# angelvillar96/STLPose

Hardware: AMD Instinct MI355X
Metric: images/sec/GPU HRNet-W32 384x288 train step; PCKh@0.5 parity (higher is better)
Workload: dtype f16/bf16; 1 GPU; HRNet-W32 384x288 bs=32/GPU train step (fwd+MSE+bwd+Adam), random-init weights; global_batch=32, parallelism=dp1

## Files before the change

stlpose_amd/csrc/conv_core.hip:

```cpp
#include <stdlib.h>
#include <algorithm>
#include <cstring>
#include <type_traits>
#include "common.cuh"

#ifndef STL_DT
#define STL_DT 2
#endif
#define STL_HAS_F32 (STL_DT == 0 || STL_DT == 2)
#define STL_HAS_BF16 (STL_DT == 1 || STL_DT == 2)
#define STL_HAS_F16 (STL_DT == 3 || STL_DT == 2)

struct ConvK {
    stl_conv p;
    int tiles_c, npt;
    int HR, HC, HP;
    int PI, pad, seff;
    int nchunks, wres;
    int cipad;
    int off_cs, off_cm, off_a, off_b, off_red;
    int sz_a, sz_b;
    int TH, TW;
    int dbg;
    float r_HC, r_TW, r_tc, r_PI, r_vp;
// ... 554 lines not shown
    STL_LAUNCH((conv_core_kernel<T, KS, WM, WN, MT, NTW, NVA, Q, PE, OCC, WR, ZM, TY, DB, EO>), grid, dim3(64 * WM * WN), lds, st, k);
    static char nbuf[160];
    static const char* nm = stl_kname<T>(nbuf, "conv_core_kernel", {KS, WM, WN, MT, NTW, NVA, Q, PE, OCC, WR, ZM, stl_code<TY>(), DB, EO});
    stl_note_kernel(nm, true);
    STL_LAUNCH_CHECK("conv_core");
    return 0;
}

struct Shape {
    int px, co, thr;
    int ws;
    int lthr, nva_max;
};
constexpr int NSHAPES = 11;
constexpr Shape SHAPES[NSHAPES] = {{128, 64, 256, 0, 256, 9}, {512, 32, 512, 0, 512, 6}, {256, 64, 512, 0, 512, 3},
                                   {256, 64, 512, 2, 512, 3}, {128, 32, 256, 0, 256, 6},
                                   {256, 64, 512, 3, 512, 3}, {128, 64, 512, 3, 512, 2}, {128, 64, 512, 1, 256, 9},
                                   {256, 32, 512, 0, 512, 3}, {128, 32, 512, 1, 256, 3}, {256, 32, 512, 3, 512, 3}};

template <typename T, typename TY, int KS, bool Q, bool PE, int EO = -1>
int dispatch(int shape, int nva, const ConvK& k, dim3 grid, size_t lds, hipStream_t st) {
    constexpr int EOC = (KS == 3 && (Q || EO == 48)) ? EO : -1;
    constexpr int EOW = (KS == 3 && EO != 48) ? EO : -1;
    switch (shape) {
        case 0:
            if (nva <= 3) return launch<T, TY, KS, 4, 1, 2, 4, 3, Q, PE>(k, grid, lds, st);
            if (nva <= 9) return launch<T, TY, KS, 4, 1, 2, 4, 9, Q, PE>(k, grid, lds, st);
            break;
        case 1:
            if (nva <= 6) return launch<T, TY, KS, 8, 1, 4, 2, 6, Q, PE>(k, grid, lds, st);
            break;
        case 2:
            if (nva <= 3) return launch<T, TY, KS, 4, 2, 4, 2, 3, Q, PE, 1>(k, grid, lds, st);
            break;
        case 3:
            if constexpr (KS == 3) {
                if (nva <= 3 && !k.wres) return launch<T, TY, KS, 4, 2, 4, 2, 3, Q, PE, 1, 0, false, true, EOC>(k, grid, lds, st);
            }
            break;
        case 8:
            if (nva <= 3 && k.wres) return launch<T, TY, KS, 8, 1, 2, 2, 3, Q, PE, 4, 1, false, false, EOC>(k, grid, lds, st);
            if (nva <= 3) return launch<T, TY, KS, 8, 1, 2, 2, 3, Q, PE, (Q ? 3 : 4)>(k, grid, lds, st);
            break;
        case 4:
            if (nva <= 3 && k.wres) return launch<T, TY, KS, 4, 1, 2, 2, 3, Q, PE, 4, 1>(k, grid, lds, st);
            if (nva <= 3) return launch<T, TY, KS, 4, 1, 2, 2, 3, Q, PE, (Q ? 3 : 4)>(k, grid, lds, st);
            if (nva <= 6) return launch<T, TY, KS, 4, 1, 2, 2, 6, Q, PE, 3>(k, grid, lds, st);
            break;
        case 7:
            if (nva <= 3) return launch_ws<T, TY, KS, 2, 4, 3, Q, (Q ? -1 : EOW)>(k, grid, lds, st);
            if (nva <= 9) return launch_ws<T, TY, KS, 2, 4, 9, Q, (Q ? -1 : EOW)>(k, grid, lds, st);
            break;
        case 9:
            if (nva <= 3) return launch_ws<T, TY, KS, 2, 2, 3, Q, EOW>(k, grid, lds, st);
            break;
    }
    return stl_set_error("conv: no kernel variant for block shape %d with %d staging vectors per thread", shape, nva);
}

static bool bnadd_shape_ok(int shape, int nva) { return nva <= 3 && (shape == 0 || shape == 2 || shape == 3 || shape == 4 || shape == 5 || shape == 6 || shape == 8 || shape == 10); }
template <typename T>
int dispatch_bnadd(int shape, int nva, const ConvK& k, dim3 grid, size_t lds, hipStream_t st) {
    if (nva <= 3) switch (shape) {
        case 0: return launch<T, T, 3, 4, 1, 2, 4, 3, true, true, 1, -1, true>(k, grid, lds, st);
        case 2:
        case 3: return launch<T, T, 3, 4, 2, 4, 2, 3, true, true, 1, -1, true>(k, grid, lds, st);
        case 4: return launch<T, T, 3, 4, 1, 2, 2, 3, true, true, 3, -1, true>(k, grid, lds, st);
        case 8: return launch<T, T, 3, 8, 1, 2, 2, 3, true, true, 3, -1, true>(k, grid, lds, st);
    }
    return stl_set_error("conv: no block-end (BNADD) variant for block shape %d with %d staging vectors per thread", shape, nva);
}

template <typename T, typename TY>
int conv_backend(int path, const stl_conv& p, const ConvK& k, int shape, int nva, dim3 grid, size_t lds, hipStream_t st) {
    const bool q = p.src.mode == STL_SRC_BNBWD;
    if constexpr (!std::is_same<T, TY>::value) {
        if (!q) return stl_set_error("conv: ydtype differs from dtype, but the launch is not a data gradient (BNBWD source)");
    }
    if constexpr (std::is_same<T, f16>::value) {
        if (q) return stl_set_error("conv: STL_F16 is a forward-tensor type; gradients are bf16 (dtype STL_BF16 + ydtype STL_F16)");
    }
    constexpr bool FWD = std::is_same<T, TY>::value, BWD = !std::is_same<T, f16>::value;
    if (path == 0) return run_1x1<T, TY>(p, st);
    if (path == 3) {
        if constexpr (sizeof(T) == 2) return dispatch_r2<T, TY>(p, k, shape == 5 ? 0 : (shape == 6 ? 1 : 2), grid, lds, st);
        return stl_set_error("conv_r2: 16-bit element types only");
    }
    if (path == 1) {
        if constexpr (FWD) return dispatch_bnadd<T>(shape, nva, k, grid, lds, st);
    }
    const bool plain = !p.bias && !p.addend && !p.mask_y && !p.mask_z && !p.red;
    const char* noeo = getenv("STL_CONV_NO_EO");
    const int eo = (noeo && (atoi(noeo) & 1)) ? -1 : epi_code(p);
    if (p.ks == 3) {
        if (q) {
            if constexpr (BWD) {
                if (eo == 1) return dispatch<T, TY, 3, true, false, 1>(shape, nva, k, grid, lds, st);
                if (eo == 7) return dispatch<T, TY, 3, true, false, 7>(shape, nva, k, grid, lds, st);
                if (eo == 2) return dispatch<T, TY, 3, true, false, 2>(shape, nva, k, grid, lds, st);
                if (eo == 0) return dispatch<T, TY, 3, true, false, 0>(shape, nva, k, grid, lds, st);
                return dispatch<T, TY, 3, true, false>(shape, nva, k, grid, lds, st);
            }
        }
        if constexpr (FWD) {
            if (plain && eo == 8) return dispatch<T, T, 3, false, true, 8>(shape, nva, k, grid, lds, st);
            if (!plain && eo == 48) return dispatch<T, T, 3, false, false, 48>(shape, nva, k, grid, lds, st);
            return plain ? dispatch<T, T, 3, false, true>(shape, nva, k, grid, lds, st) : dispatch<T, T, 3, false, false>(shape, nva, k, grid, lds, st);
        }
    }
    if (q) {
        if constexpr (BWD) return dispatch<T, TY, 1, true, false>(shape, nva, k, grid, lds, st);
    }
    if constexpr (FWD) return plain ? dispatch<T, T, 1, false, true>(shape, nva, k, grid, lds, st) : dispatch<T, T, 1, false, false>(shape, nva, k, grid, lds, st);
    return stl_set_error("conv: no kernel for this dtype combination");
}

struct Plan {
    int shape, TH, TW;
    size_t lds;
    double cost;
};

size_t lds_bytes(const stl_conv& p, int shape, int TH, int TW, int ck, ConvK* out) {
    const int taps = p.ks * p.ks, seff = p.stride;
    const int HR = (TH - 1) * seff + p.ks, HC = (TW - 1) * seff + p.ks;
    const int nchunks = ceil_div(p.Ci, ck), cipad = nchunks * ck;
    const int bco = SHAPES[shape].co, ws = SHAPES[shape].ws;
    if (ws == 3) {
        int off = 3 * cipad * 4;
        const int off_cm = off;
        off = (off + 4 * bco * 4 + 15) & ~15;
        const int off_a = off, pl = ((HR * HC * R2_PS) + 15) & ~15;
        off += 2 * pl;
        const int off_b = (off + 1023) & ~1023;
        off = off_b + bco * R2_ROWF;
        const int off_red = off;
        off += 512 * 4;
        if (out) {
            out->HR = HR, out->HC = HC, out->HP = HR * HC, out->nchunks = nchunks, out->cipad = cipad;
            out->off_cs = 0, out->off_cm = off_cm, out->off_a = off_a, out->off_b = off_b, out->off_red = off_red;
            out->sz_a = pl, out->sz_b = 0, out->wres = 0;
        }
        return (size_t)off;
    }
    int off = 3 * cipad * 4;
    const int off_cm = off;
    off += 4 * bco * 4;
    off = (off + 15) & ~15;
    const int off_a = off;
    const int sz_a = ((HR * HC * PSA) + 15) & ~15;
    off += sz_a * (ws ? 2 : 1);
    const int off_b = off;
    const int sz_b = bco * (taps * 64 + 32);
    const bool resident = nchunks == 1 || (ws == 1 && (size_t)off + (size_t)sz_b * nchunks <= 150 * 1024);
    off += resident ? sz_b * nchunks : sz_b * (ws ? 2 : 1);
    const int off_red = off_a;
    const int red = 8 * 2 * bco * 4;
    if (off - off_a < red) off = off_a + red;
    if (out) {
        out->HR = HR, out->HC = HC, out->HP = HR * HC, out->nchunks = nchunks, out->cipad = cipad;
        out->off_cs = 0, out->off_cm = off_cm, out->off_a = off_a, out->off_b = off_b, out->off_red = off_red;
        out->sz_a = ws ? sz_a : 0, out->sz_b = (ws && !resident) ? sz_b : 0;
        out->wres = resident ? 1 : 0;
    }
    return (size_t)off;
}

Plan choose_plan(const stl_conv& p, int ck) {
    Plan best{-1, 0, 0, 0, 1e300};
    const int vrows = p.B * (p.Ho + 1);
    const int r2_env = getenv("STL_CONV_R2") ? atoi(getenv("STL_CONV_R2")) : 11;
    const bool deep_small = p.stride == 1 && p.ks == 3 && p.Co >= 256 && (int64_t)p.B * p.Ho * p.Wo <= 16384 &&
                            !((r2_env & 8) && p.dtype != STL_F32 && p.Ci % 32 == 0 && p.Ci >= 64 && (r2_env & (p.src.mode == STL_SRC_BNBWD ? 2 : 1)));
    const bool want_ws = p.stride == 2 || deep_small;
    const bool wide_k = p.Co <= 32 && p.Ci >= 128 && p.stride == 1 && p.ks == 3 && !p.stuff && (int64_t)p.B * p.Ho * p.Wo >= 65536;
    const bool c32 = p.Co <= 32 && p.stride == 1 && p.ks == 3 && !wide_k;
    for (int shape = 0; shape < NSHAPES; ++shape) {
        const Shape sh = SHAPES[shape];
        if (sh.px == 0) continue;
        if (sh.px > 128 && p.stride == 2) continue;
        if ((sh.ws == 1) != want_ws) continue;
        if (want_ws && shape != (deep_small ? 9 : 7)) continue;
        if (shape == 2 || shape == 3 || shape == 5 || shape == 6) {
            static const bool db_on = !(getenv("STL_CONV_DB") && atoi(getenv("STL_CONV_DB")) == 0);
            const int r2_mode = r2_env;
            const bool db = db_on && p.ks == 3 && p.stride == 1 && p.Ci > ck;
            const bool dgrad = p.src.mode == STL_SRC_BNBWD;
            const bool r2 = db && (r2_mode & (dgrad ? 2 : 1)) && p.dtype != STL_F32 && p.Ci % 32 == 0 && p.Ci >= 64;
            const bool small_map = (r2_mode & 8) && p.Co >= 256 && (int64_t)p.B * p.Ho * p.Wo <= 16384;
            const int want = r2 ? ((dgrad || (r2_mode & 4) || small_map) ? 6 : 5) : (db ? 3 : 2);
            if (shape != want) continue;
        }
        if ((shape == 1 || shape == 8 || shape == 10) && p.Co > 32) continue;
        if ((shape == 4 || shape == 8 || shape == 10) && !c32) continue;
        if (c32 && shape != 4 && shape != 8 && shape != 10) continue;
        {
            const bool r2c32 = (r2_env & 16) && p.dtype != STL_F32 && p.Ci == 32 && (r2_env & (p.src.mode == STL_SRC_BNBWD ? 2 : 1));
            if (c32 && (shape == 8 || shape == 10) && (shape == 10) != r2c32) continue;
        }
        if (wide_k && shape != 1) continue;
        const int nblk_co = ceil_div(p.Co, sh.co);
        for (int tw = (p.Wo < 4 ? p.Wo : 4); tw <= p.Wo && tw <= sh.px; ++tw)
          for (int frac = 4; frac >= 1; --frac) {
            int th = (sh.px / tw) * frac / 4;
            if (th > vrows) th = vrows;
            if (th < 1) continue;
            const int hr = (th - 1) * p.stride + p.ks, hc = (tw - 1) * p.stride + p.ks;
            const int nva = ceil_div(hr * hc * 4, sh.lthr);
            if (nva > sh.nva_max) continue;
            const size_t lds = lds_bytes(p, shape, th, tw, ck, nullptr);
            if (shape == 4 && lds > 40 * 1024 && nva <= 3) continue;
            if (shape == 8 && lds > 80 * 1024) continue;
            if ((shape == 5 || shape == 6 || shape == 10) && lds > 76 * 1024) continue;
            if (lds > 158 * 1024) continue;
            const double tiles = (double)ceil_div(vrows, th) * ceil_div(p.Wo, tw);
            const double mfma = tiles * sh.px * sh.co * nblk_co * (double)p.Ci * p.ks * p.ks / 2048.0;
            const double bytes = tiles * nblk_co * ((double)hr * hc * p.Ci + (double)sh.co * p.ks * p.ks * p.Ci) * 2.0 / 12.0;
            const double blocks = tiles * nblk_co;
            double cost = (mfma > bytes ? mfma : bytes) + 0.3 * (mfma < bytes ? mfma : bytes);
            const double waves = blocks * sh.thr / 64.0;
            if (waves < 2048.0) cost *= 1.0 + 0.15 * (2048.0 / waves - 1.0 > 4.0 ? 4.0 : 2048.0 / waves - 1.0);
            if (c32 && shape == 4) cost *= 4.0;
            if (shape == 5 || shape == 6 || shape == 10) cost *= 0.98;
            if (cost < best.cost) best = Plan{shape, th, tw, lds, cost};
        }
    }
    return best;
}

}

#if STL_HAS_BF16
static int ydtype_of(const stl_conv& p) { return (p.dtype == STL_BF16 && p.ydtype == STL_F16) ? STL_F16 : p.dtype; }
int stl_conv_backend_bf16(int path, const stl_conv& p, const ConvK& k, int shape, int nva, dim3 grid, size_t lds, hipStream_t st) {
    if (ydtype_of(p) == STL_F16) return conv_backend<__bf16, f16>(path, p, k, shape, nva, grid, lds, st);
    return conv_backend<__bf16, __bf16>(path, p, k, shape, nva, grid, lds, st);
}
#endif
#if STL_HAS_F32
int stl_conv_backend_f32(int path, const stl_conv& p, const ConvK& k, int shape, int nva, dim3 grid, size_t lds, hipStream_t st) {
    return conv_backend<float, float>(path, p, k, shape, nva, grid, lds, st);
}
#endif
#if STL_HAS_F16
int stl_conv_backend_f16(int path, const stl_conv& p, const ConvK& k, int shape, int nva, dim3 grid, size_t lds, hipStream_t st) {
    return conv_backend<f16, f16>(path, p, k, shape, nva, grid, lds, st);
}
#endif
// ... 2 lines not shown
#ifdef STL_STAMPS
extern "C" int stl_debug_conv_stamps(long long* host12) {
    return hipMemcpyFromSymbol(host12, HIP_SYMBOL(g_stamps), 14 * sizeof(long long)) == hipSuccess ? 0 : stl_set_error("stamps: copy failed");
}
extern "C" int stl_debug_conv_stamps2(long long* host64) {
    return hipMemcpyFromSymbol(host64, HIP_SYMBOL(g_stamps2), 64 * sizeof(long long)) == hipSuccess ? 0 : stl_set_error("stamps: copy failed");
}
#endif

extern "C" int stl_conv_plan(stl_conv* pp) {
    stl_conv& p = *pp;
    STL_CHECK(p.dtype == STL_F32 || p.dtype == STL_BF16 || p.dtype == STL_F16, "conv_plan: bad dtype");
    STL_CHECK((p.ks == 1 || p.ks == 3) && (p.stride == 1 || p.stride == 2) && p.Ci > 0 && p.Co > 0, "conv_plan: bad geometry");
    const int ck = p.dtype == STL_F32 ? 16 : 32;
    Plan plan = choose_plan(p, ck);
    STL_CHECK(plan.shape >= 0, "conv_plan: no tile fits LDS for %dx%d ks %d stride %d Ci %d", p.Ho, p.Wo, p.ks, p.stride, p.Ci);
    p.shape = plan.shape, p.TH = plan.TH, p.TW = plan.TW;
    return 0;
}

extern "C" int stl_conv_bnadd_ok(const stl_conv* pp) {
    const stl_conv& p = *pp;
    if (use_1x1(p)) return 1;
    if (!(p.ks == 3 && p.stride == 1 && !p.stuff && p.shape >= 0 && p.shape < NSHAPES && p.TH > 0 && p.TW > 0)) return 0;
    const Shape sh = SHAPES[p.shape];
    const int nva = ceil_div((p.TH + 2) * (p.TW + 2) * 4, sh.lthr);
    return bnadd_shape_ok(p.shape, nva) ? 1 : 0;
}

extern "C" int stl_conv_forward(const stl_conv* pp, void* stream) {
    const stl_conv& p = *pp;
    STL_CHECK(p.dtype == STL_F32 || p.dtype == STL_BF16 || p.dtype == STL_F16, "conv: bad dtype %d", p.dtype);
    STL_CHECK(p.ydtype == 0 || p.ydtype == p.dtype || (p.dtype == STL_BF16 && p.ydtype == STL_F16), "conv: ydtype %d does not go with dtype %d", p.ydtype, p.dtype);
    STL_CHECK(p.ks == 1 || p.ks == 3, "conv: ks must be 1 or 3 (got %d)", p.ks);
    STL_CHECK(p.stride == 1 || p.stride == 2, "conv: stride must be 1 or 2");
    STL_CHECK(!(p.stuff && p.stride != 1), "conv: stuff requires stride 1");
    STL_CHECK(!(p.ks == 1 && (p.stride != 1 || p.stuff)), "conv: 1x1 must be stride 1");
    const int kv = p.dtype == STL_F32 ? 4 : 8, ck = 4 * kv;
    STL_CHECK(p.Ci % kv == 0 && p.Ci > 0, "conv: Ci=%d must be a multiple of %d", p.Ci, kv);
    STL_CHECK(p.Co % 8 == 0 && p.Co > 0, "conv: Co=%d must be a multiple of 8", p.Co);
    STL_CHECK(p.B > 0 && p.Hi > 0 && p.Wi > 0 && p.Ho > 0 && p.Wo > 0, "conv: empty tensor");
    STL_CHECK((int64_t)p.B * p.Hi * p.Wi * p.Ci < (1ll << 31) && (int64_t)p.B * p.Ho * p.Wo * p.Co < (1ll << 31),
              "conv: tensors of 2^31 or more elements are not supported");
    const int pad = p.ks == 3 ? 1 : 0;
    if (p.stuff) {
        STL_CHECK((p.Ho + 1) / 2 == p.Hi && (p.Wo + 1) / 2 == p.Wi, "conv(stuff): %dx%d is not the stride-2 image of %dx%d", p.Hi, p.Wi, p.Ho, p.Wo);
    } else {
        STL_CHECK((p.Hi + 2 * pad - p.ks) / p.stride + 1 == p.Ho && (p.Wi + 2 * pad - p.ks) / p.stride + 1 == p.Wo,
                  "conv: output %dx%d inconsistent with input %dx%d ks %d stride %d", p.Ho, p.Wo, p.Hi, p.Wi, p.ks, p.stride);
    }
    STL_CHECK(p.src.x && p.w && p.out, "conv: null tensor pointer");
    STL_CHECK(p.src.mode >= 0 && p.src.mode <= 3, "conv: bad src mode");
    const bool zm = p.src.mode == STL_SRC_BNADD;
    STL_CHECK(!zm || (((p.ks == 3 && p.stride == 1 && !p.stuff) || use_1x1(p)) && p.src.y && p.src.beta && (p.src.stats || (p.src.rmean && p.src.rvar))),
              "conv: a BNADD source needs a 3x3 stride-1 (or wide 1x1) convolution, the skip tensor in src.y and BatchNorm parameters");
    STL_CHECK(zm || !p.src_out, "conv: src_out needs a BNADD source");
    STL_CHECK(!zm || (!p.bias && !p.addend && !p.mask_y && !p.mask_z && !p.red), "conv: a BNADD source takes no epilogue operands");
    STL_CHECK(p.src.mode == STL_SRC_PLAIN || p.src.gamma, "conv: BN source without gamma");
    STL_CHECK(p.src.mode != STL_SRC_BN || p.src.beta, "conv: BN source without beta");
    STL_CHECK(p.src.mode != STL_SRC_BN || p.src.stats || (p.src.rmean && p.src.rvar), "conv: BN source without statistics");
    STL_CHECK(p.src.mode != STL_SRC_BNBWD || (p.src.y && (p.src.stats || (p.src.rmean && p.src.rvar)) && p.src.rstats), "conv: BNBWD source incomplete");
    STL_CHECK(!(p.out_stats && p.red), "conv: out_stats and red are exclusive");
    STL_CHECK(!p.red || p.mask_y, "conv: red needs mask_y");
    STL_CHECK(!p.mask_y || (p.mask_bn.gamma && p.mask_bn.beta && (p.mask_bn.stats || (p.mask_bn.rmean && p.mask_bn.rvar))), "conv: mask BN incomplete");

    const auto backend = p.dtype == STL_BF16 ? stl_conv_backend_bf16 : (p.dtype == STL_F16 ? stl_conv_backend_f16 : stl_conv_backend_f32);
    if (use_1x1(p))
        return backend(0, p, ConvK{}, 0, 0, dim3(1), 0, (hipStream_t)stream);

    Plan plan;
    if (p.shape >= 0 && p.shape < NSHAPES && p.TH > 0 && p.TW > 0) {
        STL_CHECK(p.TH * p.TW <= SHAPES[p.shape].px, "conv: tile %dx%d exceeds block shape %d", p.TH, p.TW, p.shape);
        plan = Plan{p.shape, p.TH, p.TW, 0, 0.0};
    } else if (p.TH > 0 && p.TW > 0) {
        STL_CHECK(p.TH * p.TW <= 128, "conv: explicit tile %dx%d exceeds 128 pixels", p.TH, p.TW);
        plan = Plan{0, p.TH, p.TW, 0, 0.0};
    } else {
        plan = choose_plan(p, ck);
        STL_CHECK(plan.shape >= 0, "conv: no tile fits LDS for %dx%d ks %d stride %d Ci %d", p.Ho, p.Wo, p.ks, p.stride, p.Ci);
    }
    if (plan.shape == 5 && !r2_takes(p, 0)) plan.shape = 3;
    if (plan.shape == 6 && !r2_takes(p, 1)) plan.shape = 0;
    if (plan.shape == 10 && !r2_takes(p, 2)) plan.shape = 8;
    {
        const Shape shp = SHAPES[plan.shape];
        const int nv = ceil_div(((plan.TH - 1) * p.stride + p.ks) * ((plan.TW - 1) * p.stride + p.ks) * 4, shp.lthr);
        STL_CHECK(nv <= shp.nva_max, "conv: tile %dx%d has too large a halo for block shape %d", plan.TH, plan.TW, plan.shape);
    }
    ConvK k;
    k.p = p;
    k.dbg = getenv("STL_CONV_STAMPS") ? 1 : 0;
    k.seff = p.stride;
    k.pad = pad;
    k.PI = p.stuff ? (p.Ho + 1) : p.stride * (p.Ho + 1);
    k.TH = plan.TH, k.TW = plan.TW;
    const size_t lds = lds_bytes(p, plan.shape, plan.TH, plan.TW, ck, &k);
    STL_CHECK(lds <= 160 * 1024, "conv: tile needs %zu B of LDS (>160 KiB)", lds);
    const int vrows = p.B * (p.Ho + 1);
    k.tiles_c = ceil_div(p.Wo, plan.TW);
    k.npt = ceil_div(vrows, plan.TH) * k.tiles_c;
    k.r_HC = 1.0f / k.HC, k.r_TW = 1.0f / k.TW, k.r_tc = 1.0f / k.tiles_c, k.r_PI = 1.0f / k.PI, k.r_vp = 1.0f / (p.Ho + 1);
    STL_CHECK(k.npt < (1 << 21) && (int64_t)vrows * 2 < (1 << 21) && k.HP < 4096, "conv: index range exceeds the fast-division limits");
    STL_CHECK(k.tiles_c < (1 << 11) && k.PI < (1 << 11) && p.Ho + 1 < (1 << 11), "conv: rows / columns exceed the scalar-division limits (2047)");
    {
        const unsigned long long two32 = 1ull << 32;
        k.m_tc = (two32 + k.tiles_c - 1) / k.tiles_c, k.m_PI = (two32 + k.PI - 1) / k.PI, k.m_vp = (two32 + p.Ho) / (p.Ho + 1);
    }
    STL_CHECK((int64_t)p.B * p.Hi * p.Wi < (1 << 24) && (int64_t)p.B * p.Ho * p.Wo < (1 << 24) && (int64_t)p.B * p.Hi * p.Wi * p.Ci < ((int64_t)1 << 31) &&
                  (int64_t)p.B * p.Ho * p.Wo * p.Co < ((int64_t)1 << 31),
              "conv: tensors beyond 2^24 pixels or 2^31 elements are not addressable (24-bit multiplies, 32-bit element offsets)");
    const Shape sh = SHAPES[plan.shape];
    int gx = ceil_div(k.npt, 8) * 8;
    k.ny = ceil_div(p.Co, sh.co);
    int cap = sh.thr == 512 ? 256 : 768;
    if (plan.shape == 8) cap = getenv("STL_CONV_CAP8") ? atoi(getenv("STL_CONV_CAP8")) : 432;
    if (plan.shape == 5) cap = 512;
    if (plan.shape == 6) cap = 768;
    if (plan.shape == 10) cap = getenv("STL_R2_CAP10") ? atoi(getenv("STL_R2_CAP10")) : 768;
    cap = std::max(8, (cap / k.ny + 7) / 8 * 8);
    if (const char* e = getenv("STL_CONV_GRID_CAP")) cap = atoi(e) > 0 ? (atoi(e) + 7) / 8 * 8 : cap;
    if (gx > cap) gx = cap;
    dim3 grid(gx * k.ny, 1);
    const int nva = ceil_div(k.HP * 4, sh.lthr);
    if (getenv("STL_CONV_DEBUG"))
        fprintf(stderr, "[stl conv] %dx%d Ci%d Co%d ks%d s%d: shape=%d tile=%dx%d npt=%d grid=(%d x %d) lds=%zu nva=%d nchunks=%d\n", p.Ho,
                p.Wo, p.Ci, p.Co, p.ks, p.stride, plan.shape, plan.TH, plan.TW, k.npt, gx, k.ny, lds, nva, k.nchunks);
    hipStream_t st = (hipStream_t)stream;
    return backend((plan.shape == 5 || plan.shape == 6 || plan.shape == 10) ? 3 : (zm ? 1 : 2), p, k, plan.shape, nva, grid, lds, st);
}
#endif
```

stlpose_amd/csrc/conv_r2.inc:

```
constexpr int R2_PS = 32;
constexpr int R2_ROWF = 576;

__device__ __forceinline__ void r2_dma16(const void* gsrc, char* lds_wave_uniform) {
    __builtin_amdgcn_global_load_lds((const __attribute__((address_space(1))) void*)gsrc,
                                     (__attribute__((address_space(3))) void*)lds_wave_uniform, 16, 0, 0);
}

template <typename T, typename TY, bool Q, bool ZM, int EO, int MT, int WM = 4>
__global__ __launch_bounds__(512, 4) void conv_r2_kernel(const ConvK k) {
    STAMP2(0);
    extern __shared__ __attribute__((aligned(16))) char smem[];
    constexpr int NTHR = 512, WN = 8 / WM, NTW = 2, KS = 3, TAPS = 9, BCO = 32 * WN, KV = 8, CK = 32;
    constexpr int NVA = (WM * MT * 16 == 256) ? 3 : 2;
    static_assert((WM == 4 || WM == 8) && (MT == 2 || MT == 4) && WM * MT * 16 <= 256, "128 or 256 pixels per block");
    constexpr int NDMA = BCO * TAPS * 4 / 64;
    constexpr bool PE = (EO == 8 || EO == 0);
    static_assert(sizeof(T) == 2 && sizeof(TY) == 2, "16-bit element types");
    static_assert(!ZM || Q, "block-end source: two tensors on load");
    using O = EpiOps<EO>;
    const stl_conv& p = k.p;
    const int tid = threadIdx.x, lane = tid & 63, r16 = lane & 15, g = lane >> 4;
    const int wave = __builtin_amdgcn_readfirstlane(tid >> 6);
    const int wm = wave % WM, wn = wave / WM;
    const int bl = blockIdx.x >> 3;
    const int lx = __builtin_amdgcn_readfirstlane(bl / k.ny), by = bl - lx * k.ny;
    const int n0 = by * BCO;

    float* cs = reinterpret_cast<float*>(smem + k.off_cs);
    float* cm = reinterpret_cast<float*>(smem + k.off_cm);
    char* sA = smem + k.off_a;
    char* sB = smem + k.off_b;
    float* red = reinterpret_cast<float*>(smem + k.off_red);
    const int plane = k.sz_a;

    SrcRaw raw;
    const bool need_cm = !PE && O::my(p);
    const int nitem = k.cipad + (need_cm ? BCO : 0);
    const bool it_src = tid < k.cipad;
    const int it_c = it_src ? tid : n0 + (tid - k.cipad);
    const bool it_ok = it_src ? (tid < p.Ci) : (tid < nitem && it_c < p.Co);
    if (it_ok) {
        if (it_src) {
            src_raw_load(p.src, it_c, p.Ci, raw);
        } else {
            bn_raw_load(p.mask_bn, it_c, p.Co, raw);
            raw.b = p.mask_bn.beta[it_c];
        }
    }
    auto consts_finish = [&]() __attribute__((always_inline)) {
        if (tid < nitem) {
            if (it_src) {
                float a = 0.f, b = 0.f, cc = 0.f;
                if (it_ok) src_raw_finish(p.src, raw, a, b, cc);
                cs[tid] = a, cs[k.cipad + tid] = b, cs[2 * k.cipad + tid] = cc;
            } else {
                float a = 0.f, b = 0.f, mu = 0.f, rs = 0.f;
                if (it_ok) {
                    bn_raw_finish(p.mask_bn, raw, mu, rs);
                    bn_affine(raw.g, raw.b, mu, rs, a, b);
                }
                const int c = tid - k.cipad;
                cm[c] = a, cm[BCO + c] = b, cm[2 * BCO + c] = mu, cm[3 * BCO + c] = rs;
            }
        }
        for (int item = tid + NTHR; item < nitem; item += NTHR) {
            if (item < k.cipad) {
                float a = 0.f, b = 0.f, cc = 0.f;
                if (item < p.Ci) src_consts(p.src, item, p.Ci, a, b, cc);
                cs[item] = a, cs[k.cipad + item] = b, cs[2 * k.cipad + item] = cc;
            } else {
                const int c = item - k.cipad;
                float a = 0.f, b = 0.f, mu = 0.f, rs = 0.f;
                if (n0 + c < p.Co) {
                    bn_mean_rstd(p.mask_bn, n0 + c, p.Co, mu, rs);
                    bn_affine(p.mask_bn.gamma[n0 + c], p.mask_bn.beta[n0 + c], mu, rs, a, b);
                }
                cm[c] = a, cm[BCO + c] = b, cm[2 * BCO + c] = mu, cm[3 * BCO + c] = rs;
            }
        }
    };

    auto dma_filters = [&](int k0) __attribute__((always_inline)) {
#pragma unroll
        for (int j = 0; j < (NDMA + 7) / 8; ++j) {
            const int i = wave + 8 * j;
            if (NDMA % 8 == 0 || i < NDMA) {
                int v = i * 64 + lane;
                asm volatile("" : "+v"(v));
                const int co = mulu24_vs(v, 1821) >> 16;
                const int r = v - co * 36, tap = r >> 2, part = (r & 3) ^ (((co >> 3) & 1) << 1);
                const int row = n0 + co < p.Co ? n0 + co : p.Co - 1;
                const int e = madu24_vsv(row * TAPS + tap, p.Ci, k0 + part * KV);
                r2_dma16((const char*)p.w + (size_t)(uint32_t)e * sizeof(T), sB + i * 1024);
            }
        }
    };

    const int a_part = tid & 3;
    auto tile_terms = [&](int t, int& y0, int& cb, int& b0) __attribute__((always_inline)) {
        const int tr = sdiv(t, k.m_tc), tc = t - tr * k.tiles_c;
        const int vrs = tr * k.TH * k.seff;
        cb = tc * k.TW * k.seff - k.pad;
        b0 = sdiv(vrs, k.m_PI), y0 = vrs - b0 * k.PI - k.pad;
    };
    auto slot_go = [&](int v, int y0, int cb, int b0) __attribute__((always_inline)) -> int {
        asm volatile("" : "+v"(v));
        const int hp = v >> 2, hr = fdiv(hp, k.r_HC), hc = hp - hr * k.HC;
        const int n_PI = -k.PI;
        const int iy0 = y0 + hr;
        int ix = cb + hc;
        const int wr_ = fdiv(iy0 < 0 ? 0 : iy0, k.r_PI);
        int iy = mad24_vsv(wr_, n_PI, iy0);
        bool ok = (v < k.HP * 4) & (iy0 >= 0) & (ix >= 0) & (b0 + wr_ < p.B);
        if (p.stuff) {
            ok = ok & !((iy | ix) & 1);
            iy >>= 1, ix >>= 1;
        }
        ok = ok & (iy < p.Hi) & (ix < p.Wi);
        const int e = madu24_vsv(madu24_vsv(madu24_vsv(b0 + wr_, p.Hi, iy), p.Wi, ix), p.Ci, a_part * KV);
        return ok ? e : -1;
    };
    V16 ra[NVA], rq[Q ? NVA : 1];
    int a_go[NVA];
    auto tile_setup = [&](int t) __attribute__((always_inline)) {
        int y0, cb, b0;
        tile_terms(t, y0, cb, b0);
#pragma unroll
        for (int i = 0; i < NVA; ++i) a_go[i] = slot_go(tid + i * NTHR, y0, cb, b0);
    };
    auto issue = [&](int k0, bool en) __attribute__((always_inline)) {
        const bool chok = en && (k0 + a_part * KV) < p.Ci;
#pragma unroll
        for (int i = 0; i < NVA; ++i) {
            const int off = (a_go[i] >= 0 && chok) ? a_go[i] + k0 : 0;
            ra[i] = ldg16((const char*)p.src.x + (size_t)(uint32_t)off * sizeof(T));
            if (Q) rq[i] = ldg16((const char*)p.src.y + (size_t)(uint32_t)off * sizeof(T));
        }
    };
    const float relu_lo = p.src.relu ? 0.f : -INFINITY;
    const uint32_t zown = (ZM && by == 0 && p.src_out) ? 1u : 0u;
    auto write_halo = [&](int k0) __attribute__((always_inline)) {
        const int ch = k0 + a_part * KV;
        const bool chv = ch < p.Ci;
        const int chc = chv ? ch : 0;
#pragma unroll
        for (int i = 0; i < NVA; ++i) {
            int v = tid + i * NTHR;
            asm volatile("" : "+v"(v));
            const bool ok = a_go[i] >= 0 && chv;
            V16 val = ra[i];
            if constexpr (ZM) {
                val = xform_bnadd<T>(val, rq[i], cs + chc, cs + k.cipad + chc, relu_lo);
                if (zown) {
                    const int hp = v >> 2, hr = fdiv(hp, k.r_HC), hc = hp - hr * k.HC;
                    if (ok && hr >= 1 && hr <= k.TH && hc >= 1 && hc <= k.TW) stg16((char*)p.src_out + (size_t)(a_go[i] + k0) * sizeof(T), val);
                }
            } else if constexpr (Q) {
                val = xform_bnbwd<T, TY>(val, rq[i], cs + chc, cs + k.cipad + chc, cs + 2 * k.cipad + chc);
            } else if (p.src.mode != STL_SRC_PLAIN) {
                val = xform_bn<T>(val, cs + chc, cs + k.cipad + chc, relu_lo);
            }
            mask16(val, ok);
            if (v < k.HP * 4) *reinterpret_cast<V16*>(sA + (a_part >> 1) * plane + (v >> 2) * R2_PS + (a_part & 1) * 16) = val;
        }
    };

    const int xcd = blockIdx.x & 7, nx = __builtin_amdgcn_readfirstlane((gridDim.x >> 3) / k.ny);
    const int T8 = (k.npt + 7) >> 3;
    const int vpitch = p.Ho + 1;
    const int tilepx = k.TH * k.TW;
    int it = lx, t = xcd * T8 + lx;
    bool have = (it < T8) && (t < k.npt);

    const int woff = (wn * NTW * 16 + r16) * R2_ROWF + ((g ^ (((r16 >> 3) & 1) << 1)) << 4);
    int xoff[MT];
#pragma unroll
    for (int mi = 0; mi < MT; ++mi) {
        int m = (wm * MT + mi) * 16 + r16;
        if (m >= tilepx) m = 0;
        const int ty = fdiv(m, k.r_TW), tx = m - ty * k.TW;
        xoff[mi] = (g >> 1) * plane + (ty * k.HC + tx) * R2_PS + (g & 1) * 16;
    }
    auto out_pixel = [&](int vr0, int c0, int mi, bool& pok) __attribute__((always_inline)) -> size_t {
        const int eb0 = sdiv(vr0, k.m_vp), ey0 = vr0 - eb0 * vpitch;
        int m = (wm * MT + mi) * 16 + r16;
        asm volatile("" : "+v"(m));
        const int ty = fdiv(m, k.r_TW), tx = m - ty * k.TW;
        const int oy0 = ey0 + ty, c = c0 + tx;
        const int wr_ = fdiv(oy0, k.r_vp);
        const int oy = mad24_vsv(wr_, -vpitch, oy0), b = eb0 + wr_;
        pok = (m < tilepx) & (b < p.B) & (oy < p.Ho) & (c < p.Wo);
        const int e = mulu24_vs(madu24_vsv(madu24_vsv(b, p.Ho, oy), p.Wo, c), p.Co);
        return pok ? (size_t)(uint32_t)e : 0;
    };

    if (have) {
        tile_setup(t);
        issue(0, true);
        dma_filters(0);
    }
    STAMP2(1);
    consts_finish();
    float tot = 0.f;
    f32x4 acc[MT][NTW];
#pragma unroll
    for (int mi = 0; mi < MT; ++mi)
#pragma unroll
        for (int ni = 0; ni < NTW; ++ni) acc[mi][ni] = f32x4{0.f, 0.f, 0.f, 0.f};
    __syncthreads();
    STAMP2(2);
    [[maybe_unused]] int dbg_s = 0;
    bool first = true;
    while (have) {
        const int tr = sdiv(t, k.m_tc), tc = t - tr * k.tiles_c;
        const int vr0 = tr * k.TH, c0 = tc * k.TW;
        if (!first) {
            tile_setup(t);
            issue(0, true);
        }
#pragma nounroll
        for (int ch0 = 0; ch0 < k.nchunks; ++ch0) {
            if (!first && k.nchunks > 1) dma_filters(ch0 * CK);
            first = false;
            write_halo(ch0 * CK);
            STAMP2(3 + 3 * dbg_s);
            __syncthreads();
            STAMP2(4 + 3 * dbg_s);
            if (ch0 + 1 < k.nchunks) issue((ch0 + 1) * CK, true);
            {
                constexpr int HQ = MT / 2;
                V16 wf[2][NTW], xf[2][HQ];
#pragma unroll
                for (int ni = 0; ni < NTW; ++ni) wf[0][ni] = *reinterpret_cast<const V16*>(sB + woff + ni * 16 * R2_ROWF);
#pragma unroll
                for (int q = 0; q < HQ; ++q) xf[0][q] = *reinterpret_cast<const V16*>(sA + xoff[q]);
#pragma unroll
                for (int h = 0; h < 2 * TAPS; ++h) {
                    const int tap = h >> 1, half = h & 1;
                    if (h + 1 < 2 * TAPS) {
                        const int tn = (h + 1) >> 1, hn = (h + 1) & 1;
                        const int toff = ((tn / KS) * k.HC + (tn % KS)) * R2_PS;
                        if (hn == 0) {
#pragma unroll
                            for (int ni = 0; ni < NTW; ++ni)
                                wf[tn & 1][ni] = *reinterpret_cast<const V16*>(sB + woff + ni * 16 * R2_ROWF + tn * 64);
                        }
#pragma unroll
                        for (int q = 0; q < HQ; ++q) xf[(h + 1) & 1][q] = *reinterpret_cast<const V16*>(sA + xoff[HQ * hn + q] + toff);
                    }
                    __builtin_amdgcn_sched_barrier(0);
#pragma unroll
                    for (int q = 0; q < HQ; ++q)
#pragma unroll
                        for (int ni = 0; ni < NTW; ++ni) mma16<T>(acc[HQ * half + q][ni], wf[tap & 1][ni], xf[h & 1][q]);
                    __builtin_amdgcn_sched_barrier(0);
                }
            }
            __syncthreads();
            STAMP2(5 + 3 * dbg_s);
#ifdef STL_STAMPS
            ++dbg_s;
#endif
        }
        {
            constexpr int EB = MT == 2 ? 2 : ((EO == 7 || EO < 0) ? 2 : 4);
            f2v s0[NTW][2], s1[NTW][2];
#pragma unroll
            for (int ni = 0; ni < NTW; ++ni)
#pragma unroll
                for (int h = 0; h < 2; ++h) s0[ni][h] = f2v{0.f, 0.f}, s1[ni][h] = f2v{0.f, 0.f};
            if constexpr (PE) {
#pragma unroll
                for (int mi = 0; mi < MT; ++mi) {
                    bool pok;
                    const size_t pix = out_pixel(vr0, c0, mi, pok);
                    EpiRaw<NTW> e;
                    epilogue_apply<T, NTW, BCO, true, TY, EO>(p, acc[mi], cm, pok, pix, n0, wn * NTW * 16, g, s0, s1, e);
                }
            } else {
#pragma unroll
                for (int m0 = 0; m0 < MT; m0 += EB) {
                    bool pokb[EB];
                    size_t pixb[EB];
                    EpiRaw<NTW> erb[EB];
#pragma unroll
                    for (int j = 0; j < EB; ++j) {
                        pixb[j] = out_pixel(vr0, c0, m0 + j, pokb[j]);
                        epilogue_fetch<T, NTW, true, EO>(p, pokb[j], pixb[j], n0, wn * NTW * 16, g, erb[j]);
                    }
#pragma unroll
                    for (int j = 0; j < EB; ++j)
                        epilogue_apply<T, NTW, BCO, false, TY, EO>(p, acc[m0 + j], cm, pokb[j], pixb[j], n0, wn * NTW * 16, g, s0, s1, erb[j]);
                }
            }
            STAMP2(40);
            if (O::ostats(p) || (!PE && O::red(p))) {
                xor_reduce_stats<NTW>(s0, s1);
                if (r16 == 0) {
#pragma unroll
                    for (int ni = 0; ni < NTW; ++ni)
#pragma unroll
                        for (int r = 0; r < 4; ++r) {
                            const int cl = (wn * NTW + ni) * 16 + 4 * g + r;
                            red[(wm * 2 + 0) * BCO + cl] = s0[ni][r >> 1][r & 1];
                            red[(wm * 2 + 1) * BCO + cl] = s1[ni][r >> 1][r & 1];
                        }
                }
                __syncthreads();
                if (tid < 2 * BCO) {
                    const int which = tid / BCO, cl = tid & (BCO - 1);
                    float s = 0.f;
#pragma unroll
                    for (int w = 0; w < WM; ++w) s += red[(w * 2 + which) * BCO + cl];
                    tot += s;
                }
            }
        }
        STAMP2(41);
        it += nx, t = xcd * T8 + it;
        have = (it < T8) && (t < k.npt);
    }
    double* dst = p.out_stats ? p.out_stats : p.red;
    if (dst && tid < 2 * BCO) {
        const int which = tid / BCO, cl = tid & (BCO - 1);
        if (n0 + cl < p.Co) atomicAdd(dst + (size_t)(blockIdx.x & (STL_NSHARD - 1)) * 2 * p.Co + which * p.Co + n0 + cl, (double)tot);
    }
    STAMP2(42);
}

template <typename T, typename TY, bool Q, bool ZM, int EO, int MT, int WM = 4>
int launch_r2(const ConvK& k, dim3 grid, size_t lds, hipStream_t st) {
    static bool attr_done = false;
    if (!attr_done) {
        (void)hipFuncSetAttribute(reinterpret_cast<const void*>(&conv_r2_kernel<T, TY, Q, ZM, EO, MT, WM>), hipFuncAttributeMaxDynamicSharedMemorySize, 160 * 1024);
        attr_done = true;
    }
    static const size_t lds_min = getenv("STL_R2_LDS") ? (size_t)atoi(getenv("STL_R2_LDS")) * 1024 : 0;
    if (lds < lds_min) lds = lds_min;
    STL_LAUNCH((conv_r2_kernel<T, TY, Q, ZM, EO, MT, WM>), grid, dim3(512), lds, st, k);
    static char nbuf[160];
    static const char* nm = stl_kname<T>(nbuf, "conv_r2_kernel", {stl_code<TY>(), Q, ZM, EO, MT, WM});
    stl_note_kernel(nm, true);
    STL_LAUNCH_CHECK("conv_r2");
    return 0;
}

static bool r2_takes(const stl_conv& p, int cfg) {
    if (p.dtype == STL_F32 || p.ks != 3 || p.stride != 1 || p.Ci % 32 != 0) return false;
    if (cfg == 2 ? p.Ci != 32 : p.Ci < 64) return false;
    const int eo = epi_code(p);
    if (p.src.mode == STL_SRC_BNADD) return eo == 8 || eo == 0;
    if (p.src.mode == STL_SRC_BNBWD) return cfg != 0 && p.dtype != STL_F16 && (eo == 0 || eo == 1 || eo == 2 || eo == 7);
    return eo == 8 || eo == 0 || eo == 48;
}

template <typename T, typename TY, int MT, int WM>
int dispatch_r2_cfg(const stl_conv& p, const ConvK& k, dim3 grid, size_t lds, hipStream_t st) {
    const int eo = epi_code(p);
    constexpr bool FWD = std::is_same<T, TY>::value, BWD = !std::is_same<T, f16>::value;
    if (p.src.mode == STL_SRC_BNADD) {
        if constexpr (FWD) return eo == 8 ? launch_r2<T, T, true, true, 8, MT, WM>(k, grid, lds, st) : launch_r2<T, T, true, true, 0, MT, WM>(k, grid, lds, st);
    } else if (p.src.mode == STL_SRC_BNBWD) {
        if constexpr (BWD && MT == 2) {
            switch (eo) {
                case 0: return launch_r2<T, TY, true, false, 0, MT, WM>(k, grid, lds, st);
                case 1: return launch_r2<T, TY, true, false, 1, MT, WM>(k, grid, lds, st);
                case 2: return launch_r2<T, TY, true, false, 2, MT, WM>(k, grid, lds, st);
                case 7: return launch_r2<T, TY, true, false, 7, MT, WM>(k, grid, lds, st);
            }
        }
    } else {
        if constexpr (FWD) {
            switch (eo) {
                case 8: return launch_r2<T, T, false, false, 8, MT, WM>(k, grid, lds, st);
                case 0: return launch_r2<T, T, false, false, 0, MT, WM>(k, grid, lds, st);
                case 48: return launch_r2<T, T, false, false, 48, MT, WM>(k, grid, lds, st);
            }
        }
    }
    return stl_set_error("conv_r2: no instantiation for this launch (source mode %d, operand set %d, %d x %d pixel tiles)", p.src.mode, eo, WM, MT);
}

template <typename T, typename TY>
int dispatch_r2(const stl_conv& p, const ConvK& k, int cfg, dim3 grid, size_t lds, hipStream_t st) {
    if (cfg == 0) return dispatch_r2_cfg<T, TY, 4, 4>(p, k, grid, lds, st);
    if (cfg == 1) return dispatch_r2_cfg<T, TY, 2, 4>(p, k, grid, lds, st);
    return dispatch_r2_cfg<T, TY, 2, 8>(p, k, grid, lds, st);
}
```

Baseline: 2428 images/sec.

## Add sub-pixel phase decomposition for zero-stuffed transposed 3x3 conv gradients

Adds a phase form of the r2 implicit-GEMM conv kernel for zero-stuffed (upsampling / stride-2 data-gradient) 3x3 convolutions. The kernel no longer reads the stuffed input, most of whose taps are zero. It iterates over the four output parity phases, each using only the 4, 2, 2 or 1 non-zero taps on the un-stuffed input with a smaller halo. This removes the wasted MFMA work and LDS traffic on zero entries. In exchange it quadruples the grid, adds a seek loop and a phase switch, and changes tile planning and index math, which raises the risk of subtle addressing bugs.

After: 2446 images/sec, median of 6. Within noise of the previous version (+0.7%).

```diff
diff --git a/stlpose_amd/csrc/conv_core.hip b/stlpose_amd/csrc/conv_core.hip
--- a/stlpose_amd/csrc/conv_core.hip
+++ b/stlpose_amd/csrc/conv_core.hip
@@ -660,8 +660,11 @@
     }
     constexpr bool FWD = std::is_same<T, TY>::value, BWD = !std::is_same<T, f16>::value;
     if (path == 0) return run_1x1<T, TY>(p, st);
-    if (path == 3) {
-        if constexpr (sizeof(T) == 2) return dispatch_r2<T, TY>(p, k, shape == 5 ? 0 : (shape == 6 ? 1 : 2), grid, lds, st);
+    if (path == 3 || path == 4) {
+        if constexpr (sizeof(T) == 2) {
+            const int cfg = shape == 5 ? 0 : (shape == 6 ? 1 : 2);
+            return path == 4 ? dispatch_r2_phase<T, TY>(p, k, cfg, grid, lds, st) : dispatch_r2<T, TY>(p, k, cfg, grid, lds, st);
+        }
         return stl_set_error("conv_r2: 16-bit element types only");
     }
     if (path == 1) {
@@ -699,9 +702,9 @@
     double cost;
 };
 
-size_t lds_bytes(const stl_conv& p, int shape, int TH, int TW, int ck, ConvK* out) {
+size_t lds_bytes(const stl_conv& p, int shape, int TH, int TW, int ck, ConvK* out, bool phase = false) {
     const int taps = p.ks * p.ks, seff = p.stride;
-    const int HR = (TH - 1) * seff + p.ks, HC = (TW - 1) * seff + p.ks;
+    const int HR = phase ? TH + 1 : (TH - 1) * seff + p.ks, HC = phase ? TW + 1 : (TW - 1) * seff + p.ks;
     const int nchunks = ceil_div(p.Ci, ck), cipad = nchunks * ck;
     const int bco = SHAPES[shape].co, ws = SHAPES[shape].ws;
     if (ws == 3) {
@@ -742,6 +745,24 @@
         out->wres = resident ? 1 : 0;
     }
     return (size_t)off;
+}
+
+Plan choose_phase_plan(const stl_conv& p, int ck) {
+    Plan best{-1, 0, 0, 0, 1e300};
+    const int shape = p.Co <= 32 ? 10 : 6;
+    const Shape sh = SHAPES[shape];
+    const int vrows = p.B * (p.Hi + 1);
+    for (int tw = (p.Wi < 4 ? p.Wi : 4); tw <= p.Wi && tw <= sh.px; ++tw) {
+        int th = sh.px / tw;
+        if (th > vrows) th = vrows;
+        const int halo = (th + 1) * (tw + 1);
+        if (ceil_div(halo * 4, sh.lthr) > sh.nva_max) continue;
+        const size_t lds = lds_bytes(p, shape, th, tw, ck, nullptr, true);
+        if (lds > 76 * 1024) continue;
+        const double cost = (double)ceil_div(vrows, th) * ceil_div(p.Wi, tw) + halo * 1e-6;
+        if (cost < best.cost) best = Plan{shape, th, tw, lds, cost};
+    }
+    return best;
 }
 
 Plan choose_plan(const stl_conv& p, int ck) {
@@ -910,35 +931,42 @@
     if (plan.shape == 5 && !r2_takes(p, 0)) plan.shape = 3;
     if (plan.shape == 6 && !r2_takes(p, 1)) plan.shape = 0;
     if (plan.shape == 10 && !r2_takes(p, 2)) plan.shape = 8;
+    bool phase = false;
+    if (r2_phase_takes(p) && !(getenv("STL_CONV_STUFFED") && atoi(getenv("STL_CONV_STUFFED")) != 0)) {
+        const Plan pp = choose_phase_plan(p, ck);
+        if (pp.shape >= 0) plan = pp, phase = true;
+    }
     {
         const Shape shp = SHAPES[plan.shape];
-        const int nv = ceil_div(((plan.TH - 1) * p.stride + p.ks) * ((plan.TW - 1) * p.stride + p.ks) * 4, shp.lthr);
+        const int nv = phase ? ceil_div((plan.TH + 1) * (plan.TW + 1) * 4, shp.lthr)
+                             : ceil_div(((plan.TH - 1) * p.stride + p.ks) * ((plan.TW - 1) * p.stride + p.ks) * 4, shp.lthr);
         STL_CHECK(nv <= shp.nva_max, "conv: tile %dx%d has too large a halo for block shape %d", plan.TH, plan.TW, plan.shape);
     }
     ConvK k;
     k.p = p;
     k.dbg = getenv("STL_CONV_STAMPS") ? 1 : 0;
     k.seff = p.stride;
-    k.pad = pad;
-    k.PI = p.stuff ? (p.Ho + 1) : p.stride * (p.Ho + 1);
+    k.pad = phase ? 0 : pad;
+    k.PI = phase ? (p.Hi + 1) : (p.stuff ? (p.Ho + 1) : p.stride * (p.Ho + 1));
     k.TH = plan.TH, k.TW = plan.TW;
-    const size_t lds = lds_bytes(p, plan.shape, plan.TH, plan.TW, ck, &k);
+    const size_t lds = lds_bytes(p, plan.shape, plan.TH, plan.TW, ck, &k, phase);
     STL_CHECK(lds <= 160 * 1024, "conv: tile needs %zu B of LDS (>160 KiB)", lds);
-    const int vrows = p.B * (p.Ho + 1);
-    k.tiles_c = ceil_div(p.Wo, plan.TW);
+    const int vp = (phase ? p.Hi : p.Ho) + 1;
+    const int vrows = p.B * vp;
+    k.tiles_c = ceil_div(phase ? p.Wi : p.Wo, plan.TW);
     k.npt = ceil_div(vrows, plan.TH) * k.tiles_c;
-    k.r_HC = 1.0f / k.HC, k.r_TW = 1.0f / k.TW, k.r_tc = 1.0f / k.tiles_c, k.r_PI = 1.0f / k.PI, k.r_vp = 1.0f / (p.Ho + 1);
+    k.r_HC = 1.0f / k.HC, k.r_TW = 1.0f / k.TW, k.r_tc = 1.0f / k.tiles_c, k.r_PI = 1.0f / k.PI, k.r_vp = 1.0f / vp;
     STL_CHECK(k.npt < (1 << 21) && (int64_t)vrows * 2 < (1 << 21) && k.HP < 4096, "conv: index range exceeds the fast-division limits");
     STL_CHECK(k.tiles_c < (1 << 11) && k.PI < (1 << 11) && p.Ho + 1 < (1 << 11), "conv: rows / columns exceed the scalar-division limits (2047)");
     {
         const unsigned long long two32 = 1ull << 32;
-        k.m_tc = (two32 + k.tiles_c - 1) / k.tiles_c, k.m_PI = (two32 + k.PI - 1) / k.PI, k.m_vp = (two32 + p.Ho) / (p.Ho + 1);
+        k.m_tc = (two32 + k.tiles_c - 1) / k.tiles_c, k.m_PI = (two32 + k.PI - 1) / k.PI, k.m_vp = (two32 + vp - 1) / vp;
     }
     STL_CHECK((int64_t)p.B * p.Hi * p.Wi < (1 << 24) && (int64_t)p.B * p.Ho * p.Wo < (1 << 24) && (int64_t)p.B * p.Hi * p.Wi * p.Ci < ((int64_t)1 << 31) &&
                   (int64_t)p.B * p.Ho * p.Wo * p.Co < ((int64_t)1 << 31),
               "conv: tensors beyond 2^24 pixels or 2^31 elements are not addressable (24-bit multiplies, 32-bit element offsets)");
     const Shape sh = SHAPES[plan.shape];
-    int gx = ceil_div(k.npt, 8) * 8;
+    int gx = ceil_div(k.npt, 8) * 8 * (phase ? 4 : 1);
     k.ny = ceil_div(p.Co, sh.co);
     int cap = sh.thr == 512 ? 256 : 768;
     if (plan.shape == 8) cap = getenv("STL_CONV_CAP8") ? atoi(getenv("STL_CONV_CAP8")) : 432;
@@ -954,6 +982,6 @@
         fprintf(stderr, "[stl conv] %dx%d Ci%d Co%d ks%d s%d: shape=%d tile=%dx%d npt=%d grid=(%d x %d) lds=%zu nva=%d nchunks=%d\n", p.Ho,
                 p.Wo, p.Ci, p.Co, p.ks, p.stride, plan.shape, plan.TH, plan.TW, k.npt, gx, k.ny, lds, nva, k.nchunks);
     hipStream_t st = (hipStream_t)stream;
-    return backend((plan.shape == 5 || plan.shape == 6 || plan.shape == 10) ? 3 : (zm ? 1 : 2), p, k, plan.shape, nva, grid, lds, st);
-}
-#endif
+    return backend(phase ? 4 : ((plan.shape == 5 || plan.shape == 6 || plan.shape == 10) ? 3 : (zm ? 1 : 2)), p, k, plan.shape, nva, grid, lds, st);
+}
+#endif
diff --git a/stlpose_amd/csrc/conv_r2.inc b/stlpose_amd/csrc/conv_r2.inc
--- a/stlpose_amd/csrc/conv_r2.inc
+++ b/stlpose_amd/csrc/conv_r2.inc
@@ -6,7 +6,12 @@
                                      (__attribute__((address_space(3))) void*)lds_wave_uniform, 16, 0, 0);
 }
 
-template <typename T, typename TY, bool Q, bool ZM, int EO, int MT, int WM = 4>
+constexpr int r2_ntaps(int P) { return P < 0 ? 9 : (P == 0 ? 4 : (P == 3 ? 1 : 2)); }
+constexpr int r2_tap(int P, int i) { return P < 0 ? i : (P == 0 ? (i >> 1) * 6 + (i & 1) * 2 : (P == 1 ? 1 + 6 * i : (P == 2 ? 3 + 2 * i : 4))); }
+constexpr int r2_drow(int P, int tap) { return P < 0 ? tap / 3 : (tap / 3) >> 1; }
+constexpr int r2_dcol(int P, int tap) { return P < 0 ? tap % 3 : (tap % 3) >> 1; }
+
+template <typename T, typename TY, bool Q, bool ZM, int EO, int MT, int WM = 4, bool PH = false>
 __global__ __launch_bounds__(512, 4) void conv_r2_kernel(const ConvK k) {
     STAMP2(0);
     extern __shared__ __attribute__((aligned(16))) char smem[];
@@ -17,6 +22,7 @@
     constexpr bool PE = (EO == 8 || EO == 0);
     static_assert(sizeof(T) == 2 && sizeof(TY) == 2, "16-bit element types");
     static_assert(!ZM || Q, "block-end source: two tensors on load");
+    static_assert(!PH || (!ZM && MT == 2), "phase form: data gradients, two pixel tiles per wave");
     using O = EpiOps<EO>;
     const stl_conv& p = k.p;
     const int tid = threadIdx.x, lane = tid & 63, r16 = lane & 15, g = lane >> 4;
@@ -112,7 +118,7 @@
         const int wr_ = fdiv(iy0 < 0 ? 0 : iy0, k.r_PI);
         int iy = mad24_vsv(wr_, n_PI, iy0);
         bool ok = (v < k.HP * 4) & (iy0 >= 0) & (ix >= 0) & (b0 + wr_ < p.B);
-        if (p.stuff) {
+        if (!PH && p.stuff) {
             ok = ok & !((iy | ix) & 1);
             iy >>= 1, ix >>= 1;
         }
@@ -167,10 +173,25 @@
 
     const int xcd = blockIdx.x & 7, nx = __builtin_amdgcn_readfirstlane((gridDim.x >> 3) / k.ny);
     const int T8 = (k.npt + 7) >> 3;
-    const int vpitch = p.Ho + 1;
+    const int vpitch = (PH ? p.Hi : p.Ho) + 1;
     const int tilepx = k.TH * k.TW;
-    int it = lx, t = xcd * T8 + lx;
-    bool have = (it < T8) && (t < k.npt);
+    int it = lx, t = 0, ph = 0;
+    bool have = false;
+    auto seek = [&]() __attribute__((always_inline)) {
+        if constexpr (PH) {
+            for (;;) {
+                ph = (it >= T8 ? 1 : 0) + (it >= 2 * T8 ? 1 : 0) + (it >= 3 * T8 ? 1 : 0);
+                t = xcd * T8 + it - ph * T8;
+                have = it < 4 * T8;
+                if (!have || t < k.npt) break;
+                it += nx;
+            }
+        } else {
+            t = xcd * T8 + it;
+            have = (it < T8) && (t < k.npt);
+        }
+    };
+    seek();
 
     const int woff = (wn * NTW * 16 + r16) * R2_ROWF + ((g ^ (((r16 >> 3) & 1) << 1)) << 4);
     int xoff[MT];
@@ -182,6 +203,19 @@
         xoff[mi] = (g >> 1) * plane + (ty * k.HC + tx) * R2_PS + (g & 1) * 16;
     }
     auto out_pixel = [&](int vr0, int c0, int mi, bool& pok) __attribute__((always_inline)) -> size_t {
+        if constexpr (PH) {
+            const int eb0 = sdiv(vr0, k.m_vp), ey0 = vr0 - eb0 * vpitch;
+            int m = (wm * MT + mi) * 16 + r16;
+            asm volatile("" : "+v"(m));
+            const int ty = fdiv(m, k.r_TW), tx = m - ty * k.TW;
+            const int oy0 = ey0 + ty, c = c0 + tx;
+            const int wr_ = fdiv(oy0, k.r_vp);
+            const int oy = mad24_vsv(wr_, -vpitch, oy0), b = eb0 + wr_;
+            pok = (m < tilepx) & (b < p.B) & (oy < p.Hi) & (c < p.Wi);
+            const int pa = ph < 2 ? 1 : 0, pb = (ph & 1) ? 0 : 1;
+            const int e = mulu24_vs(madu24_vsv(madu24_vsv(b, p.Ho, 2 * oy + pa), p.Wo, 2 * c + pb), p.Co);
+            return pok ? (size_t)(uint32_t)e : 0;
+        }
         const int eb0 = sdiv(vr0, k.m_vp), ey0 = vr0 - eb0 * vpitch;
         int m = (wm * MT + mi) * 16 + r16;
         asm volatile("" : "+v"(m));
@@ -194,6 +228,38 @@
         return pok ? (size_t)(uint32_t)e : 0;
     };
 
+    f32x4 acc[MT][NTW];
+    auto run_taps = [&](auto pc) __attribute__((always_inline)) {
+        constexpr int P = decltype(pc)::value, NT = r2_ntaps(P);
+        constexpr int HQ = MT / 2;
+        V16 wf[2][NTW], xf[2][HQ];
+#pragma unroll
+        for (int ni = 0; ni < NTW; ++ni) wf[0][ni] = *reinterpret_cast<const V16*>(sB + woff + ni * 16 * R2_ROWF + r2_tap(P, 0) * 64);
+#pragma unroll
+        for (int q = 0; q < HQ; ++q) xf[0][q] = *reinterpret_cast<const V16*>(sA + xoff[q]);
+#pragma unroll
+        for (int h = 0; h < 2 * NT; ++h) {
+            const int i = h >> 1, half = h & 1;
+            if (h + 1 < 2 * NT) {
+                const int in = (h + 1) >> 1, hn = (h + 1) & 1, tn = r2_tap(P, in);
+                const int toff = (r2_drow(P, tn) * k.HC + r2_dcol(P, tn)) * R2_PS;
+                if (hn == 0) {
+#pragma unroll
+                    for (int ni = 0; ni < NTW; ++ni)
+                        wf[in & 1][ni] = *reinterpret_cast<const V16*>(sB + woff + ni * 16 * R2_ROWF + tn * 64);
+                }
+#pragma unroll
+                for (int q = 0; q < HQ; ++q) xf[(h + 1) & 1][q] = *reinterpret_cast<const V16*>(sA + xoff[HQ * hn + q] + toff);
+            }
+            __builtin_amdgcn_sched_barrier(0);
+#pragma unroll
+            for (int q = 0; q < HQ; ++q)
+#pragma unroll
+                for (int ni = 0; ni < NTW; ++ni) mma16<T>(acc[HQ * half + q][ni], wf[i & 1][ni], xf[h & 1][q]);
+            __builtin_amdgcn_sched_barrier(0);
+        }
+    };
+
     if (have) {
         tile_setup(t);
         issue(0, true);
@@ -202,7 +268,6 @@
     STAMP2(1);
     consts_finish();
     float tot = 0.f;
-    f32x4 acc[MT][NTW];
 #pragma unroll
     for (int mi = 0; mi < MT; ++mi)
 #pragma unroll
@@ -227,34 +292,15 @@
             __syncthreads();
             STAMP2(4 + 3 * dbg_s);
             if (ch0 + 1 < k.nchunks) issue((ch0 + 1) * CK, true);
-            {
-                constexpr int HQ = MT / 2;
-                V16 wf[2][NTW], xf[2][HQ];
-#pragma unroll
-                for (int ni = 0; ni < NTW; ++ni) wf[0][ni] = *reinterpret_cast<const V16*>(sB + woff + ni * 16 * R2_ROWF);
-#pragma unroll
-                for (int q = 0; q < HQ; ++q) xf[0][q] = *reinterpret_cast<const V16*>(sA + xoff[q]);
-#pragma unroll
-                for (int h = 0; h < 2 * TAPS; ++h) {
-                    const int tap = h >> 1, half = h & 1;
-                    if (h + 1 < 2 * TAPS) {
-                        const int tn = (h + 1) >> 1, hn = (h + 1) & 1;
-                        const int toff = ((tn / KS) * k.HC + (tn % KS)) * R2_PS;
-                        if (hn == 0) {
-#pragma unroll
-                            for (int ni = 0; ni < NTW; ++ni)
-                                wf[tn & 1][ni] = *reinterpret_cast<const V16*>(sB + woff + ni * 16 * R2_ROWF + tn * 64);
-                        }
-#pragma unroll
-                        for (int q = 0; q < HQ; ++q) xf[(h + 1) & 1][q] = *reinterpret_cast<const V16*>(sA + xoff[HQ * hn + q] + toff);
-                    }
-                    __builtin_amdgcn_sched_barrier(0);
-#pragma unroll
-                    for (int q = 0; q < HQ; ++q)
-#pragma unroll
-                        for (int ni = 0; ni < NTW; ++ni) mma16<T>(acc[HQ * half + q][ni], wf[tap & 1][ni], xf[h & 1][q]);
-                    __builtin_amdgcn_sched_barrier(0);
-                }
+            if constexpr (PH) {
+                switch (ph) {
+                    case 0: run_taps(std::integral_constant<int, 0>{}); break;
+                    case 1: run_taps(std::integral_constant<int, 1>{}); break;
+                    case 2: run_taps(std::integral_constant<int, 2>{}); break;
+                    default: run_taps(std::integral_constant<int, 3>{}); break;
+                }
+            } else {
+                run_taps(std::integral_constant<int, -1>{});
             }
             __syncthreads();
             STAMP2(5 + 3 * dbg_s);
@@ -317,8 +363,8 @@
             }
         }
         STAMP2(41);
-        it += nx, t = xcd * T8 + it;
-        have = (it < T8) && (t < k.npt);
+        it += nx;
+        seek();
     }
     double* dst = p.out_stats ? p.out_stats : p.red;
     if (dst && tid < 2 * BCO) {
@@ -328,18 +374,18 @@
     STAMP2(42);
 }
 
-template <typename T, typename TY, bool Q, bool ZM, int EO, int MT, int WM = 4>
+template <typename T, typename TY, bool Q, bool ZM, int EO, int MT, int WM = 4, bool PH = false>
 int launch_r2(const ConvK& k, dim3 grid, size_t lds, hipStream_t st) {
     static bool attr_done = false;
     if (!attr_done) {
-        (void)hipFuncSetAttribute(reinterpret_cast<const void*>(&conv_r2_kernel<T, TY, Q, ZM, EO, MT, WM>), hipFuncAttributeMaxDynamicSharedMemorySize, 160 * 1024);
+        (void)hipFuncSetAttribute(reinterpret_cast<const void*>(&conv_r2_kernel<T, TY, Q, ZM, EO, MT, WM, PH>), hipFuncAttributeMaxDynamicSharedMemorySize, 160 * 1024);
         attr_done = true;
     }
     static const size_t lds_min = getenv("STL_R2_LDS") ? (size_t)atoi(getenv("STL_R2_LDS")) * 1024 : 0;
     if (lds < lds_min) lds = lds_min;
-    STL_LAUNCH((conv_r2_kernel<T, TY, Q, ZM, EO, MT, WM>), grid, dim3(512), lds, st, k);
+    STL_LAUNCH((conv_r2_kernel<T, TY, Q, ZM, EO, MT, WM, PH>), grid, dim3(512), lds, st, k);
     static char nbuf[160];
-    static const char* nm = stl_kname<T>(nbuf, "conv_r2_kernel", {stl_code<TY>(), Q, ZM, EO, MT, WM});
+    static const char* nm = stl_kname<T>(nbuf, "conv_r2_kernel", {stl_code<TY>(), Q, ZM, EO, MT, WM, PH});
     stl_note_kernel(nm, true);
     STL_LAUNCH_CHECK("conv_r2");
     return 0;
@@ -387,3 +433,38 @@
     if (cfg == 1) return dispatch_r2_cfg<T, TY, 2, 4>(p, k, grid, lds, st);
     return dispatch_r2_cfg<T, TY, 2, 8>(p, k, grid, lds, st);
 }
+
+static bool r2_phase_takes(const stl_conv& p) {
+    if (!p.stuff || p.dtype != STL_BF16 || p.ks != 3 || p.stride != 1 || p.Ci % 32 != 0) return false;
+    if (p.Ci < 64) return false;
+    if ((p.Ho & 1) || (p.Wo & 1) || p.Hi * 2 != p.Ho || p.Wi * 2 != p.Wo) return false;
+    const int eo = epi_code(p);
+    const bool same = p.ydtype == 0 || p.ydtype == p.dtype;
+    if (p.src.mode == STL_SRC_BNBWD) return eo == 0 || eo == 1 || eo == 2 || (eo == 7 && !(same && p.Co <= 32));
+    return p.src.mode == STL_SRC_PLAIN && eo == 0 && same;
+}
+
+template <typename T, typename TY, int WM>
+int dispatch_r2_phase_cfg(const stl_conv& p, const ConvK& k, dim3 grid, size_t lds, hipStream_t st) {
+    if constexpr (std::is_same<T, __bf16>::value) {
+        const int eo = epi_code(p);
+        if (p.src.mode == STL_SRC_BNBWD) {
+            switch (eo) {
+                case 0: return launch_r2<T, TY, true, false, 0, 2, WM, true>(k, grid, lds, st);
+                case 1: return launch_r2<T, TY, true, false, 1, 2, WM, true>(k, grid, lds, st);
+                case 2: return launch_r2<T, TY, true, false, 2, 2, WM, true>(k, grid, lds, st);
+                case 7:
+                    if constexpr (!(WM == 8 && std::is_same<T, TY>::value)) return launch_r2<T, TY, true, false, 7, 2, WM, true>(k, grid, lds, st);
+                    break;
+            }
+        } else if constexpr (std::is_same<T, TY>::value) {
+            if (eo == 0) return launch_r2<T, T, false, false, 0, 2, WM, true>(k, grid, lds, st);
+        }
+    }
+    return stl_set_error("conv_r2: no phase-form instantiation for this launch (source mode %d, operand set %d)", p.src.mode, epi_code(p));
+}
+
+template <typename T, typename TY>
+int dispatch_r2_phase(const stl_conv& p, const ConvK& k, int cfg, dim3 grid, size_t lds, hipStream_t st) {
+    return cfg == 1 ? dispatch_r2_phase_cfg<T, TY, 4>(p, k, grid, lds, st) : dispatch_r2_phase_cfg<T, TY, 8>(p, k, grid, lds, st);
+}
```
